# marian42/shapegan

Measured on AMD Instinct MI355X. Metric: GAN train steps/sec @32^3 voxels (train_wgan.py 5 critic + 1 generator updates, batch 64/GPU), higher is better.
Workload: dtype f32; 1 GPU; train_wgan.py 32^3 voxel WGAN, fp32, batch=64 synthetic SDF grids (BASELINE configs[1]); global_batch=64, per_gpu_batch=64, parallelism=dp1

## Files before the change

### shapegan_amd/csrc/conv3d_halo.hip

```cpp
#include "conv_common.h"

#ifndef SG_RING
#define SG_RING 8
#endif
#ifndef SG_ABLATE
#define SG_ABLATE 0
#endif

namespace sg {

constexpr int kHD = 4, kHH = 18, kHWF = 18;
constexpr int kHWH = 10;
constexpr int kROWH = 2 * kHWH;
constexpr int kROWD = kHH * kROWH;
constexpr int kHS = kHD * kROWD;
constexpr int kCC = 4;

struct HaloFwdArgs {
    const float* x;
    const float4* wp;
    const float* bias;
    float* y;
    ConvGeom g;
    int Cin, Cout;
// ... 567 lines not shown

    const int tid = threadIdx.x, lane = tid & 63;
    const int wave = __builtin_amdgcn_readfirstlane(tid >> 6);
    const int wm = R32 ? 0 : wave >> 1, wn = wave & 1, r = lane & 31, kpar = lane >> 5;
    const int tnf = R32 ? wave >> 1 : 0;
    const int lpart = MODE == 0 ? (r >> 3) * BX::BW + (r & 7) : (r >> 4) * BX::PL + ((r >> 2) & 3) * BX::BW + (r & 3);
    const int lanebase = wn * BX::WNOFF + tnf * BX::TNOFF + lpart + 1 - kpar;

    f32x16 acc[NTN];
#pragma unroll
    for (int t = 0; t < NTN; ++t)
#pragma unroll
        for (int q = 0; q < 16; ++q) acc[t][q] = 0.f;

    lds_float* const bl = (lds_float*)box;
    const lds_float* bb[2][kDCC];
#pragma unroll
    for (int b = 0; b < 2; ++b)
#pragma unroll
        for (int c = 0; c < kDCC; ++c) {
            bb[b][c] = bl + b * kDBUF + c * kDB + lanebase;
            pin_vgpr(bb[b][c]);
        }
    lds_float* sdst = bl + tid;
    pin_vgpr(sdst);

    const int G = a.Cout;
    const int par0 = blockIdx.z * a.ppw, par_end = par0 + a.ppw;
    const unsigned par_bytes = (unsigned)(a.mtiles * 2) * (unsigned)G * 1024u;
    const __amdgpu_buffer_rsrc_t wres = make_rsrc(a.wp + ((long)(R32 ? blockIdx.y : blockIdx.y * 2 + wm) * G) * 64);
    const unsigned wvoff = lane * 16;

    const int O3 = a.g.OD * a.g.OH * a.g.OW;
    const int obias = (a.g.OH + 1) * a.g.OW + 1;
    const __amdgpu_buffer_rsrc_t dres = __builtin_amdgcn_make_buffer_rsrc(
        const_cast<float*>(a.dy + (long)n * a.g.Cy * O3 - obias), 0, 1 << 26, 0x00020000);
    const unsigned chan_bytes = (unsigned)O3 * 4u;
    unsigned gword[kDNF], goff[kDNF];
#pragma unroll
    for (int f = 0; f < kDNF; ++f) {
        const int e = tid + 256 * f;
        const int ci = e / kDB;
        int rem = e - ci * kDB, smp = 0;
        if (MODE == 1) {
            smp = rem / 125;
            rem -= smp * 125;
        }
        const int hd = rem / BX::PL, hh = (rem - hd * BX::PL) / BX::BW, hw = rem % BX::BW;
        const int od = qd0 - 1 + hd, oh = qh0 - 1 + hh, ow = qw0 - 1 + hw;
        const bool never = e >= kDCC * kDB || (int)n + smp >= a.batch;
        const unsigned cls = (od < 0 ? 1u << 26 : 0u) | (od + 1 >= a.g.OD ? 1u << 27 : 0u) | (oh < 0 ? 1u << 28 : 0u) |
                             (oh + 1 >= a.g.OH ? 1u << 29 : 0u) | (ow < 0 ? 1u << 30 : 0u) | (ow + 1 >= a.g.OW ? 1u << 31 : 0u);
        const int off0 = (smp * a.g.Cy + ci) * O3 + (od * a.g.OH + oh) * a.g.OW + ow + obias;
        gword[f] = never ? 0xffffffffu : ((unsigned)off0 * 4u) | cls;
        pin_vgpr(gword[f]);
    }
    unsigned pshift = 0;
    auto set_goff = [&](int par) __attribute__((always_inline)) {
        const int pd = (par >> 2) & 1, ph = (par >> 1) & 1, pw = par & 1;
        const unsigned mask = 0x03ffffffu | (pd ? 1u << 27 : 1u << 26) | (ph ? 1u << 29 : 1u << 28) | (pw ? 1u << 31 : 1u << 30);
#pragma unroll
        for (int f = 0; f < kDNF; ++f) goff[f] = gword[f] & mask;
        pshift = (unsigned)((pd * a.g.OH + ph) * a.g.OW + pw) * 4u;
    };
    const long I3 = (long)a.g.ID * a.g.IH * a.g.IW;
    const int nn = MODE == 0 ? (int)n : (int)n + wn;
    const __amdgpu_buffer_rsrc_t ores = make_rsrc(a.dx + (long)(nn < a.batch ? nn : 0) * a.g.Cx * I3);
    const __amdgpu_buffer_rsrc_t bres = make_rsrc(a.bias ? a.bias : a.dx);
    unsigned ovoff[NTN];
#pragma unroll
    for (int tn = 0; tn < NTN; ++tn) {
        int qd, qh, qw;
        if (MODE == 0) {
            qd = qd0 + wn;
            qh = qh0 + (tnf + tn) * 4 + (r >> 3);
            qw = qw0 + (r & 7);
        } else {
            qd = 2 * (tnf + tn) + (r >> 4);
            qh = (r >> 2) & 3;
            qw = r & 3;
        }
        ovoff[tn] = (unsigned)(((2 * qd) * a.g.IH + 2 * qh) * a.g.IW + 2 * qw + 4 * kpar * (int)I3) * 4u;
        pin_vgpr(ovoff[tn]);
    }
    const unsigned bvoff = kpar * 16;
#ifdef SG_DGRAD_NO_PAIR
    const bool paired = false;
#else
    const bool paired = a.ppw >= 2;
#endif
    float keep[NTN][16];
#pragma unroll
    for (int t = 0; t < NTN; ++t)
#pragma unroll
        for (int q = 0; q < 16; ++q) keep[t][q] = 0.f;
    auto write_parity = [&](int par) __attribute__((always_inline)) {
        const int pd = (par >> 2) & 1, ph = (par >> 1) & 1, pw = par & 1;
        const unsigned oshift = (unsigned)((pd * a.g.IH + ph) * a.g.IW) * 4u;
        if (nn < a.batch) {
            if (paired && pw == 0) {
#pragma unroll
                for (int q = 0; q < 16; ++q) {
                    const int cis = ci0 + wm * 32 + (q & 3) + 8 * (q >> 2);
                    const float bv = a.bias && cis < a.Cin ? buf_load(bres, bvoff, (unsigned)cis * 4u) : 0.f;
#pragma unroll
                    for (int tn = 0; tn < NTN; ++tn) keep[tn][q] = sg_apply_act(acc[tn][q] + bv, a.act, a.slope);
                }
            } else if (paired) {
                typedef unsigned u32x2 __attribute__((ext_vector_type(2)));
#pragma unroll
                for (int q = 0; q < 16; ++q) {
                    const int cis = ci0 + wm * 32 + (q & 3) + 8 * (q >> 2);
                    if (cis < a.Cin) {
                        const float bv = a.bias ? buf_load(bres, bvoff, (unsigned)cis * 4u) : 0.f;
#pragma unroll
                        for (int tn = 0; tn < NTN; ++tn) {
                            u32x2 v;
                            v.x = __builtin_bit_cast(unsigned, keep[tn][q]);
                            v.y = __builtin_bit_cast(unsigned, sg_apply_act(acc[tn][q] + bv, a.act, a.slope));
                            __builtin_amdgcn_raw_buffer_store_b64(v, ores, (int)ovoff[tn], (int)((unsigned)cis * (unsigned)I3 * 4u + oshift), 0);
                        }
                    }
                }
            } else {
#pragma unroll
                for (int q = 0; q < 16; ++q) {
                    const int cis = ci0 + wm * 32 + (q & 3) + 8 * (q >> 2);
                    if (cis < a.Cin) {
                        const float bv = a.bias ? buf_load(bres, bvoff, (unsigned)cis * 4u) : 0.f;
#pragma unroll
                        for (int tn = 0; tn < NTN; ++tn) {
                            const float v = sg_apply_act(acc[tn][q] + bv, a.act, a.slope);
                            __builtin_amdgcn_raw_buffer_store_b32(__builtin_bit_cast(unsigned, v), ores, (int)ovoff[tn],
                                                                  (int)((unsigned)cis * (unsigned)I3 * 4u + oshift + 4u * pw), 0);
                        }
                    }
                }
            }
        }
#pragma unroll
        for (int t = 0; t < NTN; ++t)
#pragma unroll
            for (int q = 0; q < 16; ++q) acc[t][q] = 0.f;
    };

    set_goff(par0);
    float fv[kDNF];
    constexpr int kRing = 8;
    float4 aring[kRing];
    unsigned wcur = (unsigned)par0 * par_bytes;
#pragma unroll
    for (int f = 0; f < kDNF; ++f) fv[f] = buf_load(dres, goff[f], pshift);
#pragma unroll
    for (int u = 0; u < kRing; ++u) aring[u] = buf_load4(wres, wvoff, wcur + (unsigned)u * 1024u);
#pragma unroll
    for (int f = 0; f < kDNF; ++f) sdst[256 * f] = fv[f];
    __syncthreads();

    constexpr int O00 = BX::PL + BX::BW, O01 = BX::PL, O10 = BX::BW, O11 = 0;
    const int nstage = a.Cout / kDCC;
    auto stage = [&](auto tag, unsigned dys, unsigned wnext) __attribute__((always_inline)) {
        constexpr int CUR = decltype(tag)::value, NXT = CUR ^ 1;
        float bq[NTN][4];
#pragma unroll
        for (int tn = 0; tn < NTN; ++tn) {
            const lds_float* hb = bb[CUR][0] + tn * BX::TNOFF;
            bq[tn][0] = hb[O00];
            bq[tn][1] = hb[O01];
            bq[tn][2] = hb[O10];
            bq[tn][3] = hb[O11];
        }
        __builtin_amdgcn_sched_barrier(0);
#pragma unroll
        for (int c = 0; c < kDCC; ++c) {
            const float4 a_cur = aring[c % kRing];
            aring[c % kRing] = c + kRing < kDCC ? buf_load4(wres, wvoff, wcur + (unsigned)(c + kRing) * 1024u)
                                                : buf_load4(wres, wvoff, wnext + (unsigned)(c + kRing - kDCC) * 1024u);
            float b[NTN][4];
#pragma unroll
            for (int tn = 0; tn < NTN; ++tn)
#pragma unroll
                for (int j = 0; j < 4; ++j) b[tn][j] = bq[tn][j];
            if (c + 1 < kDCC) {
#pragma unroll
                for (int tn = 0; tn < NTN; ++tn) {
                    const lds_float* hb = bb[CUR][c + 1] + tn * BX::TNOFF;
                    bq[tn][0] = hb[O00];
                    bq[tn][1] = hb[O01];
                    bq[tn][2] = hb[O10];
                    bq[tn][3] = hb[O11];
                }
            }
            if (c < kDCC / 2) {
#pragma unroll
                for (int f = 2 * c; f < 2 * c + 2; ++f) fv[f] = buf_load(dres, goff[f], dys + pshift);
            } else {
#pragma unroll
                for (int f = 2 * (c - kDCC / 2); f < 2 * (c - kDCC / 2) + 2; ++f) sdst[NXT * kDBUF + 256 * f] = fv[f];
            }
            __builtin_amdgcn_sched_barrier(0);
            const float av[4] = {a_cur.x, a_cur.y, a_cur.z, a_cur.w};
#pragma unroll
            for (int j = 0; j < 4; ++j)
#pragma unroll
                for (int tn = 0; tn < NTN; ++tn) acc[tn] = __builtin_amdgcn_mfma_f32_32x32x2f32(av[j], b[tn][j], acc[tn], 0, 0, 0);
            __builtin_amdgcn_sched_barrier(0);
        }
        wcur = wnext;
        __syncthreads();
    };
    for (int par = par0; par < par_end; ++par) {
        const bool more = par + 1 < par_end;
        const unsigned wlast = more ? (unsigned)(par + 1) * par_bytes : (unsigned)par * par_bytes + (unsigned)(nstage - 1) * kDCC * 1024u;
        const unsigned dlast = more ? 0u : (unsigned)(nstage - 1) * kDCC * chan_bytes;
        int s = 0;
        for (; s + 1 < nstage; s += 2) {
            stage(IntTag<0>(), (unsigned)(s + 1) * kDCC * chan_bytes, wcur + kDCC * 1024u);
            const bool last = s + 2 == nstage;
            if (last && more) set_goff(par + 1);
            stage(IntTag<1>(), last ? dlast : (unsigned)(s + 2) * kDCC * chan_bytes, last ? wlast : wcur + kDCC * 1024u);
        }
        if (s < nstage) stage(IntTag<0>(), dlast, wlast);
        write_parity(par);
    }
}

template <int MODE>
__global__ void __launch_bounds__(256) conv_dgrad_halo_kernel(HaloDgradArgs a) {
    conv_dgrad_halo_body<MODE, false>(a);
}
template <int MODE>
__global__ void __launch_bounds__(256) conv_dgrad_halo32_kernel(HaloDgradArgs a) {
    conv_dgrad_halo_body<MODE, true>(a);
}

size_t halo_dgrad_workspace_bytes(int Cin, int Cout) { return (size_t)8 * ((Cin + 63) / 64) * 64 * Cout * 8 * sizeof(float); }

int halo_dgrad_try(const float* dy, const float* w, const float* bias, float* dx, int batch, int Cin, int Cin_total,
                   const ConvGeom& g, int Cout, int act, float slope, void* workspace, size_t workspace_bytes,
                   hipStream_t stream, int force, bool packed_already, PackJobs* collect) {
    const bool mode1 = g.OD == 4 && g.OH == 4 && g.OW == 4;
    if (!mode1 && (g.OW % 8 != 0 || g.OH % 8 != 0 || g.OD % 2 != 0)) return 0;
    if (Cout % 16 != 0 || Cin < 32 || Cin % 8 != 0) return 0;
    if (((long)2 * g.Cy * g.OD * g.OH * g.OW + (long)(g.OH + 1) * g.OW + 1) * 4 >= (1L << 26)) return 0;
    if (!workspace || workspace_bytes < halo_dgrad_workspace_bytes(Cin, Cout)) return 0;
    if ((long)batch * g.Cy * g.OD * g.OH * g.OW >= (1L << 31)) return 0;
    if ((long)2 * g.Cy * g.OD * g.OH * g.OW * 4 >= (long)kBufRange || (long)Cout * 1024 >= (long)kBufRange) return 0;
    const int ntw = mode1 ? 1 : g.OW / 8, nth = mode1 ? 1 : g.OH / 8, ntd = mode1 ? 1 : g.OD / 2;
    const long tiles = mode1 ? (batch + 1) / 2 : (long)batch * ntd * nth * ntw;
    const int mtiles = (Cin + 63) / 64;
    if (!force && tiles * mtiles * 8 < (mode1 ? 16 : 64)) return 0;
    if (tiles >= (1L << 31) || mtiles > 65535) return 0;
    float4* wp = (float4*)workspace;
    if ((long)8 * mtiles * 2 * Cout * 1024 >= (long)kBufRange) return 0;
    if (collect) return collect->add(1, w, wp, Cout, Cin_total, Cin, mtiles * 2);
    if (!packed_already) {
        const long total = 8L * mtiles * 2 * Cout * 64;
        int blocks = (int)((total + 255) / 256);
        if (blocks > 4096) blocks = 4096;
        hipLaunchKernelGGL(pack_dgrad_frag_kernel, dim3(blocks), dim3(256), 0, stream, w, wp, Cout, Cin_total, Cin, mtiles * 2);
    }
    HaloDgradArgs a;
    a.dy = dy;
    a.wp = wp;
    a.bias = bias;
    a.dx = dx;
    a.g = g;
    a.Cin = Cin;
    a.Cout = Cout;
    a.mtiles = mtiles;
    a.batch = batch;
    a.dntw = FastDiv(ntw);
    a.dnth = FastDiv(nth);
    a.dntd = FastDiv(ntd);
    a.act = act;
    a.slope = slope;
    int ppw = 8;
    while (ppw > 1 && (tiles * mtiles * (8 / ppw) < 512 || (force & 2) || (Cout / 16) % 2 != 0)) ppw >>= 1;
    if ((force >> 2) && (Cout / 16) % 2 == 0) ppw = force >> 2;
    if ((long)8 * mtiles * 2 * Cout * 1024 >= (long)kBufRange) return 0;
    a.ppw = ppw;
    size_t lds = (size_t)2 * 16 * 256 * sizeof(float);
    {
        const long wgs = tiles * mtiles * (8 / ppw);
        const long cost2 = ((wgs + 511) / 512) * 2, cost3 = ((wgs + 767) / 768) * 3;
        if (cost2 <= cost3) lds = 56 * 1024;
    }
    const bool r32 = Cin <= 32 || tiles * mtiles * (8 / ppw) < 256;
    const dim3 grid((unsigned)tiles, r32 ? (unsigned)((Cin + 31) / 32) : (unsigned)mtiles, 8 / ppw);
    if (mode1 && r32)
        hipLaunchKernelGGL((conv_dgrad_halo32_kernel<1>), grid, dim3(256), lds, stream, a);
    else if (mode1)
        hipLaunchKernelGGL((conv_dgrad_halo_kernel<1>), grid, dim3(256), lds, stream, a);
    else if (r32)
        hipLaunchKernelGGL((conv_dgrad_halo32_kernel<0>), grid, dim3(256), lds, stream, a);
    else
        hipLaunchKernelGGL((conv_dgrad_halo_kernel<0>), grid, dim3(256), lds, stream, a);
    return 1;
}

constexpr int kWROWD = 368;
constexpr int kWHS = kHD * kWROWD;
constexpr int kWNF = (2 * kHD * kHH + 7) / 8;

struct HaloWgradArgs {
    const float4* ap;
    const float* x;
    float* ws;
    ConvGeom g;
    int Cin, Cout, nslice, per_split, mt_total;
    long ldw;
    FastDiv dntw, dnth, dOD;
};

__global__ void __launch_bounds__(256) pack_wgrad_dy_kernel(const float* __restrict__ dy, float4* __restrict__ ap,
                                                            ConvGeom g, int Cout, int MT, int nslice, FastDiv dntw,
                                                            FastDiv dnth, FastDiv dOD) {
    const long total = (long)MT * nslice * 8 * 64;
    const long O3 = (long)g.OD * g.OH * g.OW;
    for (long e = (long)blockIdx.x * 256 + threadIdx.x; e < total; e += (long)gridDim.x * 256) {
        const int lane = (int)(e & 63);
        const int gq = (int)((e >> 6) & 7);
        const long q = e >> 9;
        const uint32_t sl = (uint32_t)(q % nslice);
        const int mt = (int)(q / nslice);
        uint32_t twi, thi, od, n, q1, q2;
        dntw.divmod(sl, q1, twi);
        dnth.divmod(q1, q2, thi);
        dOD.divmod(q2, n, od);
        const int co = mt * 32 + (lane & 31);
        float4 v = make_float4(0.f, 0.f, 0.f, 0.f);
        if (co < Cout) {
            const float* src = dy + ((long)n * Cout + co) * O3 + ((long)od * g.OH + (thi * 8 + gq)) * g.OW + twi * 8 + (lane >> 5);
            v = make_float4(src[0], src[2], src[4], src[6]);
        }
        ap[e] = v;
    }
}

template <int NCH>
__global__ void __launch_bounds__(256) conv_wgrad_halo_kernel(HaloWgradArgs a) {
    extern __shared__ __attribute__((aligned(16))) float wbox[];
    const int tid = threadIdx.x, lane = tid & 63;
    const int wave = __builtin_amdgcn_readfirstlane(tid >> 6);
    const int wm = NCH == 2 ? wave >> 1 : 0, wn = NCH == 2 ? wave & 1 : wave, r = lane & 31, kpar = lane >> 5;
    const int ci0 = blockIdx.x * NCH;
    const int mt0 = blockIdx.y * (NCH == 2 ? 4 : 2);
    constexpr int NF = NCH == 2 ? kWNF : 2 * kWNF;
    constexpr int NV = NCH == 2 ? kWNF : kWNF / 2;
    const int split = blockIdx.z;
    const int s_beg = split * a.per_split, s_end = min(a.nslice, s_beg + a.per_split);

    int lanebase[2];
#pragma unroll
    for (int tn = 0; tn < 2; ++tn) {
        const int col = wn * 64 + tn * 32 + r;
        const int tap = col & 63, kd = tap >> 4, kh = (tap >> 2) & 3, kw = tap & 3;
        lanebase[tn] = (col >> 6) * kWHS + kd * kWROWD + kh * kROWH + (kw & 1) * kHWH + (kw >> 1) + kpar;
    }

    f32x16 acc[2][2];
#pragma unroll
    for (int i = 0; i < 2; ++i)
#pragma unroll
        for (int j = 0; j < 2; ++j)
#pragma unroll
            for (int q = 0; q < 16; ++q) acc[i][j][q] = 0.f;

    const int I3 = a.g.ID * a.g.IH * a.g.IW;
    const int fl_w = tid & 31, frow = tid >> 5;
    const int lds_w = (fl_w & 1) * kHWH + (fl_w >> 1);
    const int prow = (tid >> 1) % (kHD * kHH);
    const int pad = (prow / kHH) * kWROWD + (prow % kHH) * kROWH + (tid & 1) * kHWH + (kHWH - 1);
    lds_float* const wl = (lds_float*)wbox;
    lds_float* sdst[kWNF / 2];
    unsigned voff[NV], cls[NV];
#pragma unroll
    for (int f = 0; f < kWNF / 2; ++f) {
        const int row = 8 * f + frow;
        const int hd = row / kHH, hh = row - hd * kHH;
        const bool inbox = fl_w < kHWF && row < kHD * kHH;
        sdst[f] = wl + (inbox ? hd * kWROWD + hh * kROWH + lds_w : pad);
        pin_vgpr(sdst[f]);
#pragma unroll
        for (int c = 0; c < (NCH == 2 ? 2 : 1); ++c) {
            const bool ok = inbox && (ci0 + c) < a.Cin;
            voff[c * (kWNF / 2) + f] = ok ? (unsigned)(c * I3 + (hd * a.g.IH + hh) * a.g.IW + fl_w) * 4u : kBufOutside;
            cls[c * (kWNF / 2) + f] = (hd == 0 ? 1u << 26 : 0u) | (hd == kHD - 1 ? 1u << 27 : 0u) | (hh == 0 ? 1u << 28 : 0u) |
                                      (hh == kHH - 1 ? 1u << 29 : 0u) | (fl_w == 0 ? 1u << 30 : 0u) |
                                      (fl_w == kHWF - 1 ? 1u << 31 : 0u);
            pin_vgpr(voff[c * (kWNF / 2) + f]);
            pin_vgpr(cls[c * (kWNF / 2) + f]);
        }
    }
    float fv[NF];
    unsigned eoff[NV];
    __amdgpu_buffer_rsrc_t xres;
    auto xres_of = [&]() __attribute__((always_inline)) { return xres; };
    const unsigned chan_bytes = (unsigned)I3 * 4u;
    auto copy_load = [&](int f) __attribute__((always_inline)) {
        if constexpr (NCH == 2) {
            return buf_load(xres_of(), eoff[f], 0);
        } else {
            return buf_load(xres_of(), eoff[f % (kWNF / 2)], (unsigned)(f / (kWNF / 2)) * chan_bytes);
        }
    };
    const int ntw_ = (int)a.g.OW / 8, nth_ = (int)a.g.OH / 8;
    auto copy_prepare = [&](int sl) {
        uint32_t twi, thi, od, n, q1, q2;
        a.dntw.divmod((uint32_t)sl, q1, twi);
        a.dnth.divmod(q1, q2, thi);
        a.dOD.divmod(q2, n, od);
        const long origin = ((long)n * a.g.Cx + ci0) * I3 + ((2 * (long)od - 1) * a.g.IH + (16 * (long)thi - 1)) * a.g.IW +
                            (16 * (long)twi - 1);
        xres = __builtin_amdgcn_make_buffer_rsrc(const_cast<float*>(a.x + origin), 0, 1 << 26, 0x00020000);
        const unsigned flags = (od == 0 ? 1u << 26 : 0u) | ((int)od == a.g.OD - 1 ? 1u << 27 : 0u) | (thi == 0 ? 1u << 28 : 0u) |
                               ((int)thi == nth_ - 1 ? 1u << 29 : 0u) | (twi == 0 ? 1u << 30 : 0u) |
                               ((int)twi == ntw_ - 1 ? 1u << 31 : 0u);
#pragma unroll
        for (int f = 0; f < NV; ++f) eoff[f] = (cls[f] & flags) | voff[f];
    };

    const int nst = s_end - s_beg;
    constexpr int kRing = 8;
    const int G = nst * 8;
    if (nst > 0) {
        __amdgpu_buffer_rsrc_t ares[2];
#pragma unroll
        for (int t = 0; t < 2; ++t) ares[t] = make_rsrc(a.ap + ((long)(mt0 + wm * 2 + t) * a.nslice + s_beg) * 8 * 64);
        const unsigned avoff = lane * 16;
        const lds_float* bb[2][2][2];
#pragma unroll
        for (int b = 0; b < 2; ++b)
#pragma unroll
            for (int tn = 0; tn < 2; ++tn)
#pragma unroll
                for (int h = 0; h < 2; ++h) {
                    bb[b][tn][h] = wl + b * (NCH * kWHS) + lanebase[tn] + h * (8 * kROWH);
                    pin_vgpr(bb[b][tn][h]);
                }

        copy_prepare(s_beg);
#pragma unroll
        for (int f = 0; f < NF; ++f) fv[f] = copy_load(f);
        float4 aring[kRing][2];
#pragma unroll
        for (int u = 0; u < kRing; ++u)
#pragma unroll
            for (int t = 0; t < 2; ++t) aring[u][t] = buf_load4(ares[t], avoff, (unsigned)(u < G ? u : G - 1) * 1024u);
#pragma unroll
        for (int f = 0; f < NF; ++f) sdst[f % (kWNF / 2)][(f / (kWNF / 2)) * kWHS] = fv[f];
        __syncthreads();

        auto stage = [&](auto tag, int st) {
            constexpr int CUR = decltype(tag)::value, NXT = CUR ^ 1;
            const int snext = st + 1 < nst ? st + 1 : st;
            float bq[2][4];
#pragma unroll
            for (int tn = 0; tn < 2; ++tn) {
                const lds_float* hb = bb[CUR][tn][0];
                bq[tn][0] = hb[0];
                bq[tn][1] = hb[2];
                bq[tn][2] = hb[4];
                bq[tn][3] = hb[6];
            }
            copy_prepare(s_beg + snext);
            __builtin_amdgcn_sched_barrier(0);
#pragma unroll
            for (int gq = 0; gq < 8; ++gq) {
                float4 a_cur[2];
#pragma unroll
                for (int t = 0; t < 2; ++t) a_cur[t] = aring[gq][t];
                int gi = (st + 1) * 8 + gq;
                gi = gi < G ? gi : G - 1;
#pragma unroll
                for (int t = 0; t < 2; ++t) aring[gq][t] = buf_load4(ares[t], avoff, (unsigned)gi * 1024u);
                float b[2][4];
#pragma unroll
                for (int tn = 0; tn < 2; ++tn)
#pragma unroll
                    for (int j = 0; j < 4; ++j) b[tn][j] = bq[tn][j];
                if (gq + 1 < 8) {
#pragma unroll
                    for (int tn = 0; tn < 2; ++tn) {
                        const lds_float* hb = bb[CUR][tn][(gq + 1) >> 2] + 2 * ((gq + 1) & 3) * kROWH;
                        bq[tn][0] = hb[0];
                        bq[tn][1] = hb[2];
                        bq[tn][2] = hb[4];
                        bq[tn][3] = hb[6];
                    }
                }
#pragma unroll
                for (int f = 0; f < NF; ++f) {
                    if (f * 4 / NF == gq) fv[f] = copy_load(f);
                    if (f * 4 / NF + 4 == gq) sdst[f % (kWNF / 2)][NXT * (NCH * kWHS) + (f / (kWNF / 2)) * kWHS] = fv[f];
                }
                __builtin_amdgcn_sched_barrier(0);
#pragma unroll
                for (int j = 0; j < 4; ++j) {
                    const float a0 = j == 0 ? a_cur[0].x : (j == 1 ? a_cur[0].y : (j == 2 ? a_cur[0].z : a_cur[0].w));
                    const float a1 = j == 0 ? a_cur[1].x : (j == 1 ? a_cur[1].y : (j == 2 ? a_cur[1].z : a_cur[1].w));
                    acc[0][0] = __builtin_amdgcn_mfma_f32_32x32x2f32(a0, b[0][j], acc[0][0], 0, 0, 0);
                    acc[1][0] = __builtin_amdgcn_mfma_f32_32x32x2f32(a1, b[0][j], acc[1][0], 0, 0, 0);
                    acc[0][1] = __builtin_amdgcn_mfma_f32_32x32x2f32(a0, b[1][j], acc[0][1], 0, 0, 0);
                    acc[1][1] = __builtin_amdgcn_mfma_f32_32x32x2f32(a1, b[1][j], acc[1][1], 0, 0, 0);
                }
                __builtin_amdgcn_sched_barrier(0);
            }
            __syncthreads();
        };
        for (int st = 0; st + 1 < nst; st += 2) {
            stage(IntTag<0>(), st);
            stage(IntTag<1>(), st + 1);
        }
        if (nst & 1) stage(IntTag<0>(), nst - 1);
    }

    float* out = a.ws + (long)split * a.Cout * a.ldw;
#pragma unroll
    for (int tn = 0; tn < 2; ++tn) {
        const int col = wn * 64 + tn * 32 + r;
        const int ci = ci0 + (col >> 6);
        if (ci >= a.Cin) continue;
        const long cbase = (long)ci * 64 + (col & 63);
#pragma unroll
        for (int t = 0; t < 2; ++t) {
#pragma unroll
            for (int q = 0; q < 16; ++q) {
                const int co = (mt0 + wm * 2 + t) * 32 + (q & 3) + 8 * (q >> 2) + 4 * kpar;
                if (co < a.Cout) out[(long)co * a.ldw + cbase] = acc[t][tn][q];
            }
        }
    }
}

__global__ void __launch_bounds__(256) pack_wgrad_dy4_kernel(const float* __restrict__ dy, float4* __restrict__ ap, int Cout,
                                                             int MT, int nslice) {
    const long total = (long)MT * nslice * 8 * 64;
    for (long e = (long)blockIdx.x * 256 + threadIdx.x; e < total; e += (long)gridDim.x * 256) {
        const int lane = (int)(e & 63);
        const int gq = (int)((e >> 6) & 7);
        const long q = e >> 9;
        const long sl = q % nslice;
        const int mt = (int)(q / nslice);
        const int co = mt * 32 + (lane & 31);
        float4 v = make_float4(0.f, 0.f, 0.f, 0.f);
        if (co < Cout) {
            const float* src = dy + (sl * Cout + co) * 64 + (gq >> 1) * 16 + (gq & 1) * 8 + (lane >> 5);
            v = make_float4(src[0], src[2], src[4], src[6]);
        }
        ap[e] = v;
    }
}

__global__ void __launch_bounds__(256) conv_wgrad_halo4_kernel(HaloWgradArgs a) {
    constexpr int kBUF = 2 * k4CH;
    extern __shared__ __attribute__((aligned(16))) float wbox[];
    lds_float* const wl = (lds_float*)wbox;
    const int tid = threadIdx.x, lane = tid & 63;
    const int wave = __builtin_amdgcn_readfirstlane(tid >> 6);
    const int wm = wave >> 1, wn = wave & 1, r = lane & 31, kpar = lane >> 5;
    const int ci0 = blockIdx.x * 2, mt0 = blockIdx.y * 4, split = blockIdx.z;
    const int s_beg = split * a.per_split, s_end = min(a.nslice, s_beg + a.per_split);
    const int nst = s_end - s_beg;

    f32x16 acc[2][2];
#pragma unroll
    for (int i = 0; i < 2; ++i)
#pragma unroll
        for (int j = 0; j < 2; ++j)
#pragma unroll
            for (int q = 0; q < 16; ++q) acc[i][j][q] = 0.f;

    for (int e = tid; e < 2 * kBUF; e += 256) wl[e] = 0.f;

    if (nst > 0) {
        const lds_float* bb[2][2][4];
#pragma unroll
        for (int tn = 0; tn < 2; ++tn) {
            const int tap = tn * 32 + r, kd = tap >> 4, kh = (tap >> 2) & 3, kw = tap & 3;
            const int lb = wn * k4CH + kd * k4PLANE + kh * k4ROW + (kw & 1) * k4HALF + (kw >> 1) + kpar;
#pragma unroll
            for (int b = 0; b < 2; ++b)
#pragma unroll
                for (int od = 0; od < 4; ++od) {
                    bb[b][tn][od] = wl + b * kBUF + lb + od * (2 * k4PLANE);
                    pin_vgpr(bb[b][tn][od]);
                }
        }
        unsigned voff[4];
        lds_float* sdst[4];
#pragma unroll
        for (int f = 0; f < 4; ++f) {
            const int e = tid + 256 * f, c = e >> 9, idx = e & 511;
            const int id = idx >> 6, ih = (idx >> 3) & 7, iw = idx & 7;
            voff[f] = (ci0 + c) < a.Cin ? (unsigned)e * 4u : kBufOutside;
            sdst[f] = wl + c * k4CH + (id + 1) * k4PLANE + (ih + 1) * k4ROW + ((iw + 1) & 1) * k4HALF + ((iw + 1) >> 1);
            pin_vgpr(voff[f]);
            pin_vgpr(sdst[f]);
        }
        __amdgpu_buffer_rsrc_t ares[2];
#pragma unroll
        for (int t = 0; t < 2; ++t) ares[t] = make_rsrc(a.ap + ((long)(mt0 + wm * 2 + t) * a.nslice + s_beg) * 8 * 64);
        const unsigned avoff = lane * 16;
        const long slice_floats = (long)a.g.Cx * 512;
        const float* xb = a.x + (long)s_beg * slice_floats + (long)ci0 * 512;
        const int G = nst * 8;
        constexpr int kRing = 8;
        float fv[4];
        __syncthreads();
        {
            const __amdgpu_buffer_rsrc_t xres = make_rsrc(xb);
#pragma unroll
            for (int f = 0; f < 4; ++f) fv[f] = buf_load(xres, voff[f], 0);
        }
        float4 aring[kRing][2];
#pragma unroll
        for (int u = 0; u < kRing; ++u)
#pragma unroll
            for (int t = 0; t < 2; ++t) aring[u][t] = buf_load4(ares[t], avoff, (unsigned)(u < G ? u : G - 1) * 1024u);
#pragma unroll
        for (int f = 0; f < 4; ++f) *sdst[f] = fv[f];
        __syncthreads();

        auto stage = [&](auto tag, int st) {
            constexpr int CUR = decltype(tag)::value, NXT = CUR ^ 1;
            const int snext = st + 1 < nst ? st + 1 : st;
            const __amdgpu_buffer_rsrc_t xres = make_rsrc(xb + (long)snext * slice_floats);
            float bq[2][4];
#pragma unroll
            for (int tn = 0; tn < 2; ++tn) {
                const lds_float* hb = bb[CUR][tn][0];
                bq[tn][0] = hb[0];
                bq[tn][1] = hb[2];
                bq[tn][2] = hb[2 * k4ROW];
                bq[tn][3] = hb[2 * k4ROW + 2];
            }
            __builtin_amdgcn_sched_barrier(0);
#pragma unroll
            for (int gq = 0; gq < 8; ++gq) {
                float4 a_cur[2];
#pragma unroll
                for (int t = 0; t < 2; ++t) a_cur[t] = aring[gq][t];
                int gi = (st + 1) * 8 + gq;
                gi = gi < G ? gi : G - 1;
#pragma unroll
                for (int t = 0; t < 2; ++t) aring[gq][t] = buf_load4(ares[t], avoff, (unsigned)gi * 1024u);
                float b[2][4];
#pragma unroll
                for (int tn = 0; tn < 2; ++tn)
#pragma unroll
                    for (int j = 0; j < 4; ++j) b[tn][j] = bq[tn][j];
                if (gq + 1 < 8) {
#pragma unroll
                    for (int tn = 0; tn < 2; ++tn) {
                        const lds_float* hb = bb[CUR][tn][(gq + 1) >> 1] + ((gq + 1) & 1) * (4 * k4ROW);
                        bq[tn][0] = hb[0];
                        bq[tn][1] = hb[2];
                        bq[tn][2] = hb[2 * k4ROW];
                        bq[tn][3] = hb[2 * k4ROW + 2];
                    }
                }
                if (gq < 4) fv[gq] = buf_load(xres, voff[gq], 0);
                else sdst[gq - 4][NXT * kBUF] = fv[gq - 4];
                __builtin_amdgcn_sched_barrier(0);
#pragma unroll
                for (int j = 0; j < 4; ++j) {
                    const float a0 = j == 0 ? a_cur[0].x : (j == 1 ? a_cur[0].y : (j == 2 ? a_cur[0].z : a_cur[0].w));
                    const float a1 = j == 0 ? a_cur[1].x : (j == 1 ? a_cur[1].y : (j == 2 ? a_cur[1].z : a_cur[1].w));
                    acc[0][0] = __builtin_amdgcn_mfma_f32_32x32x2f32(a0, b[0][j], acc[0][0], 0, 0, 0);
                    acc[1][0] = __builtin_amdgcn_mfma_f32_32x32x2f32(a1, b[0][j], acc[1][0], 0, 0, 0);
                    acc[0][1] = __builtin_amdgcn_mfma_f32_32x32x2f32(a0, b[1][j], acc[0][1], 0, 0, 0);
                    acc[1][1] = __builtin_amdgcn_mfma_f32_32x32x2f32(a1, b[1][j], acc[1][1], 0, 0, 0);
                }
                __builtin_amdgcn_sched_barrier(0);
            }
            __syncthreads();
        };
        for (int st = 0; st + 1 < nst; st += 2) {
            stage(IntTag<0>(), st);
            stage(IntTag<1>(), st + 1);
        }
        if (nst & 1) stage(IntTag<0>(), nst - 1);
    }

    float* out = a.ws + (long)split * a.Cout * a.ldw;
#pragma unroll
    for (int tn = 0; tn < 2; ++tn) {
        const int col = wn * 64 + tn * 32 + r;
        const int ci = ci0 + (col >> 6);
        if (ci >= a.Cin) continue;
        const long cbase = (long)ci * 64 + (col & 63);
#pragma unroll
        for (int t = 0; t < 2; ++t) {
#pragma unroll
            for (int q = 0; q < 16; ++q) {
                const int co = (mt0 + wm * 2 + t) * 32 + (q & 3) + 8 * (q >> 2) + 4 * kpar;
                if (co < a.Cout) out[(long)co * a.ldw + cbase] = acc[t][tn][q];
            }
        }
    }
}

__global__ void __launch_bounds__(256) wgrad_halo_finalize_kernel(const float* __restrict__ ws, float* __restrict__ dw,
                                                                  int Cout, int ncol, long ldw, int nsplit) {
    const long total = (long)Cout * ncol, total4 = total >> 2;
    for (long e4 = (long)blockIdx.x * 256 + threadIdx.x; e4 < total4; e4 += (long)gridDim.x * 256) {
        const f32x4* p = reinterpret_cast<const f32x4*>(ws) + e4;
        f32x4 v = {0.f, 0.f, 0.f, 0.f};
        int s = 0;
        for (; s + 3 < nsplit; s += 4) {
            const f32x4 a0 = p[(long)s * total4], a1 = p[(long)(s + 1) * total4], a2 = p[(long)(s + 2) * total4],
                        a3 = p[(long)(s + 3) * total4];
            v += a0;
            v += a1;
            v += a2;
            v += a3;
        }
        for (; s < nsplit; ++s) v += p[(long)s * total4];
        const long e = e4 << 2;
        const long co = e / ncol, c = e - co * ncol;
        *reinterpret_cast<f32x4*>(dw + co * ldw + c) = v;
    }
}

static bool wgrad_mode4(const ConvGeom& g) { return g.OD == 4 && g.OH == 4 && g.OW == 4; }

static bool wgrad_rows64(const ConvGeom& g, int Cin, int Cout) {
    return !wgrad_mode4(g) && Cout <= 64 && Cin >= 4 && Cin % 4 == 0;
}
static void wgrad_halo_plan(int batch, const ConvGeom& g, int Cin, int Cout, int& nslice, int& nsplit, int& mtiles) {
    nslice = wgrad_mode4(g) ? batch : batch * g.OD * (g.OH / 8) * (g.OW / 8);
    const bool rows64 = wgrad_rows64(g, Cin, Cout);
    mtiles = rows64 ? (Cout + 63) / 64 : (Cout + 127) / 128;
    const int ntiles = (rows64 ? Cin / 4 : (Cin + 1) / 2) * mtiles;
    nsplit = (512 + ntiles - 1) / ntiles;
    if (nsplit > nslice / 4) nsplit = nslice / 4 > 0 ? nslice / 4 : 1;
    if (nsplit < 1) nsplit = 1;
}

size_t halo_wgrad_workspace_bytes(int batch, int Cin, int Cout, int OD, int OH, int OW) {
    if ((OH % 8 != 0 || OW % 8 != 0) && !(OD == 4 && OH == 4 && OW == 4)) return 0;
    ConvGeom g;
    g.OD = OD;
    g.OH = OH;
    g.OW = OW;
    int nslice, nsplit, mtiles;
    g.ID = 2 * OD;
    g.IH = 2 * OH;
    g.IW = 2 * OW;
    wgrad_halo_plan(batch, g, Cin, Cout, nslice, nsplit, mtiles);
    const size_t pack = (size_t)mtiles * 4 * nslice * 8 * 64 * sizeof(float4);
    const size_t part = (size_t)nsplit * Cout * Cin * 64 * sizeof(float);
    return pack + part + 256;
}

int halo_wgrad_dy_image_plan(int batch, int Cin, int Cout, const ConvGeom& g, size_t workspace_bytes, int* mt_total, long* nslice_out) {
    const bool mode4 = wgrad_mode4(g);
    if (!(mode4 || (g.OD == 8 && g.OH == 8 && g.OW == 8)) || Cout % 128 != 0 || Cin < 2) return 0;
    if ((long)batch * g.Cx * g.ID * g.IH * g.IW >= (1L << 31) || (long)2 * g.ID * g.IH * g.IW * 4 >= (1L << 26)) return 0;
    int nslice, nsplit, mtiles;
    wgrad_halo_plan(batch, g, Cin, Cout, nslice, nsplit, mtiles);
    const int ntiles = ((Cin + 1) / 2) * mtiles;
    if (Cout <= 64 || (long)ntiles * nsplit < 384) return 0;
    if (workspace_bytes < halo_wgrad_workspace_bytes(batch, Cin, Cout, g.OD, g.OH, g.OW)) return 0;
    *mt_total = mtiles * 4;
    *nslice_out = nslice;
    return 1;
}

__global__ void __launch_bounds__(256) act_bwd_pack8_kernel(const float* __restrict__ y, const float* __restrict__ dy,
                                                            float* __restrict__ dz, float* __restrict__ rowsum,
                                                            float4* __restrict__ ap, long rows, int C, long nslice, int act, float slope) {
    const long row = (long)blockIdx.x * 4 + (threadIdx.x >> 6);
    if (row >= rows) return;
    const int lane = threadIdx.x & 63;
    const long base = row * 512 + lane * 8;
    const f32x4 y0 = *reinterpret_cast<const f32x4*>(y + base), y1 = *reinterpret_cast<const f32x4*>(y + base + 4);
    const f32x4 g0 = *reinterpret_cast<const f32x4*>(dy + base), g1 = *reinterpret_cast<const f32x4*>(dy + base + 4);
    f32x4 z0, z1;
#pragma unroll
    for (int j = 0; j < 4; ++j) {
        z0[j] = act == SG_ACT_LEAKY ? (y0[j] > 0.f ? g0[j] : g0[j] * slope) : (y0[j] > 0.f ? g0[j] : 0.f);
        z1[j] = act == SG_ACT_LEAKY ? (y1[j] > 0.f ? g1[j] : g1[j] * slope) : (y1[j] > 0.f ? g1[j] : 0.f);
    }
    *reinterpret_cast<f32x4*>(dz + base) = z0;
    *reinterpret_cast<f32x4*>(dz + base + 4) = z1;
    const float s = sg_wave_sum(((z0[0] + z0[1]) + (z0[2] + z0[3])) + ((z1[0] + z1[1]) + (z1[2] + z1[3])));
    if (lane == 0) rowsum[row] = s;
    const long n = row / C;
    const int co = (int)(row - n * C), mt = co >> 5, r = co & 31, od = lane >> 3, oh = lane & 7;
    const long e = (((long)mt * nslice + n * 8 + od) * 8 + oh) * 64 + r;
    ap[e] = make_float4(z0[0], z0[2], z1[0], z1[2]);
    ap[e + 32] = make_float4(z0[1], z0[3], z1[1], z1[3]);
}
int halo_act_bwd_pack8_launch(const float* y, const float* dy, float* dz, float* rowsum, void* ap, long rows, int C, long nslice,
                              int act, float slope, hipStream_t stream) {
    hipLaunchKernelGGL(act_bwd_pack8_kernel, dim3((unsigned)((rows + 3) / 4)), dim3(256), 0, stream, y, dy, dz, rowsum, (float4*)ap,
                       rows, C, nslice, act, slope);
    return 1;
}

int halo_wgrad_try(const float* dy, const float* x, float* dw, int batch, int Cin, int Cin_total, const ConvGeom& g, int Cout,
                   void* workspace, size_t workspace_bytes, hipStream_t stream, int force, bool dy_packed) {
    const bool mode4 = wgrad_mode4(g);
    if ((!mode4 && (g.OW % 8 != 0 || g.OH % 8 != 0)) || Cin < 2 || Cout < 32) return 0;
    if ((long)batch * g.Cx * g.ID * g.IH * g.IW >= (1L << 31)) return 0;
    if ((long)2 * g.ID * g.IH * g.IW * 4 >= (1L << 26)) return 0;
    int nslice, nsplit, mtiles;
    wgrad_halo_plan(batch, g, Cin, Cout, nslice, nsplit, mtiles);
    const bool rows64 = wgrad_rows64(g, Cin, Cout) && (long)4 * g.ID * g.IH * g.IW * 4 < (1L << 26);
    if (wgrad_rows64(g, Cin, Cout) && !rows64) return 0;
    const int ntiles = (rows64 ? Cin / 4 : (Cin + 1) / 2) * mtiles;
    if (!force && ((Cout <= 64 && !rows64) || (long)ntiles * nsplit < 384)) return 0;
    const size_t need = halo_wgrad_workspace_bytes(batch, Cin, Cout, g.OD, g.OH, g.OW);
    if (!workspace || workspace_bytes < need) return 0;
    const int per_split = (nslice + nsplit - 1) / nsplit;
    nsplit = (nslice + per_split - 1) / per_split;

    const FastDiv dntw(mode4 ? 1 : g.OW / 8), dnth(mode4 ? 1 : g.OH / 8), dOD(g.OD);
    float4* ap = (float4*)workspace;
    const size_t pack_floats4 = (size_t)mtiles * 4 * nslice * 8 * 64;
    float* part = (float*)(ap + pack_floats4);
    if (!dy_packed) {
        int blocks = (int)((pack_floats4 + 255) / 256);
        if (blocks > 8192) blocks = 8192;
        if (mode4)
            hipLaunchKernelGGL(pack_wgrad_dy4_kernel, dim3(blocks), dim3(256), 0, stream, dy, ap, Cout, mtiles * 4, nslice);
        else
            hipLaunchKernelGGL(pack_wgrad_dy_kernel, dim3(blocks), dim3(256), 0, stream, dy, ap, g, Cout, rows64 ? mtiles * 2 : mtiles * 4,
                               nslice, dntw, dnth, dOD);
    }
    HaloWgradArgs a;
    a.ap = ap;
    a.x = x;
    a.g = g;
    a.Cin = Cin;
    a.Cout = Cout;
    a.nslice = nslice;
    a.per_split = per_split;
    a.mt_total = rows64 ? mtiles * 2 : mtiles * 4;
    a.dntw = dntw;
    a.dnth = dnth;
    a.dOD = dOD;
    const bool direct = nsplit == 1;
    a.ws = direct ? dw : part;
    a.ldw = direct ? (long)Cin_total * 64 : (long)Cin * 64;
    if (mode4) {
        hipLaunchKernelGGL(conv_wgrad_halo4_kernel, dim3((Cin + 1) / 2, mtiles, nsplit), dim3(256),
                           (size_t)2 * 2 * k4CH * sizeof(float), stream, a);
    } else {
        if (rows64) {
            const size_t lds = (size_t)2 * 4 * kWHS * sizeof(float);
            hipLaunchKernelGGL(conv_wgrad_halo_kernel<4>, dim3(Cin / 4, mtiles, nsplit), dim3(256), lds, stream, a);
        } else {
            const size_t lds = (size_t)2 * 2 * kWHS * sizeof(float);
            hipLaunchKernelGGL(conv_wgrad_halo_kernel<2>, dim3((Cin + 1) / 2, mtiles, nsplit), dim3(256), lds, stream, a);
        }
    }
    if (!direct) {
        const long total = (long)Cout * Cin * 64;
        int fb = (int)((total / 4 + 255) / 256);
        if (fb > 2048) fb = 2048;
        hipLaunchKernelGGL(wgrad_halo_finalize_kernel, dim3(fb), dim3(256), 0, stream, (const float*)part, dw, Cout, Cin * 64,
                           (long)Cin_total * 64, nsplit);
    }
    return 1;
}

}
```

Before: 60.34 steps/s.

## Remap wgrad columns so waves skip padding-only MFMA steps statically

Reorders the weight-gradient GEMM column-to-tap mapping in the halo wgrad kernels so that each wave-pair owns a fixed group of kernel-depth taps. This lets the boundary steps that touch only zero padding be skipped at compile time: both their LDS B loads and their MFMAs are dropped. The 2-channel path gets a specialised variant for OH==8, with a smaller LDS row stride and boundary flags folded into the buffer offsets. The mode-4 kernel is always specialised this way. The cost is two instantiated bodies per kernel with a wave-level branch, plus remapped output indexing that must stay correct.

```diff
diff --git a/shapegan_amd/csrc/conv3d_halo.hip b/shapegan_amd/csrc/conv3d_halo.hip
--- a/shapegan_amd/csrc/conv3d_halo.hip
+++ b/shapegan_amd/csrc/conv3d_halo.hip
@@ -893,6 +893,7 @@
 constexpr int kWROWD = 368;
 constexpr int kWHS = kHD * kWROWD;
 constexpr int kWNF = (2 * kHD * kHH + 7) / 8;
+constexpr int kWROWD_SKIP = 364;
 
 struct HaloWgradArgs {
     const float4* ap;
@@ -929,12 +930,16 @@
     }
 }
 
-template <int NCH>
-__global__ void __launch_bounds__(256) conv_wgrad_halo_kernel(HaloWgradArgs a) {
+template <int NCH, int V>
+__device__ __forceinline__ void conv_wgrad_halo_body(const HaloWgradArgs& a) {
+    constexpr bool SKIP = V >= 0;
+    static_assert(!SKIP || NCH == 2, "the static-skip column map is the 2-channel form's");
+    constexpr int WROWD = SKIP ? kWROWD_SKIP : kWROWD;
+    constexpr int WHS = kHD * WROWD;
     extern __shared__ __attribute__((aligned(16))) float wbox[];
     const int tid = threadIdx.x, lane = tid & 63;
     const int wave = __builtin_amdgcn_readfirstlane(tid >> 6);
-    const int wm = NCH == 2 ? wave >> 1 : 0, wn = NCH == 2 ? wave & 1 : wave, r = lane & 31, kpar = lane >> 5;
+    const int wm = NCH == 2 ? wave >> 1 : 0, wn = SKIP ? V : (NCH == 2 ? wave & 1 : wave), r = lane & 31, kpar = lane >> 5;
     const int ci0 = blockIdx.x * NCH;
     const int mt0 = blockIdx.y * (NCH == 2 ? 4 : 2);
     constexpr int NF = NCH == 2 ? kWNF : 2 * kWNF;
@@ -942,12 +947,13 @@
     const int split = blockIdx.z;
     const int s_beg = split * a.per_split, s_end = min(a.nslice, s_beg + a.per_split);
 
+    auto col_ci = [&](int tn) { return SKIP ? r >> 4 : (wn * 64 + tn * 32 + r) >> 6; };
+    auto col_tap = [&](int tn) { return SKIP ? ((r >> 2) & 3) * 16 + (2 * wn + tn) * 4 + (r & 3) : (tn * 32 + r) & 63; };
     int lanebase[2];
 #pragma unroll
     for (int tn = 0; tn < 2; ++tn) {
-        const int col = wn * 64 + tn * 32 + r;
-        const int tap = col & 63, kd = tap >> 4, kh = (tap >> 2) & 3, kw = tap & 3;
-        lanebase[tn] = (col >> 6) * kWHS + kd * kWROWD + kh * kROWH + (kw & 1) * kHWH + (kw >> 1) + kpar;
+        const int tap = col_tap(tn), kd = tap >> 4, kh = (tap >> 2) & 3, kw = tap & 3;
+        lanebase[tn] = col_ci(tn) * WHS + kd * WROWD + kh * kROWH + (kw & 1) * kHWH + (kw >> 1) + kpar;
     }
 
     f32x16 acc[2][2];
@@ -962,7 +968,7 @@
     const int fl_w = tid & 31, frow = tid >> 5;
     const int lds_w = (fl_w & 1) * kHWH + (fl_w >> 1);
     const int prow = (tid >> 1) % (kHD * kHH);
-    const int pad = (prow / kHH) * kWROWD + (prow % kHH) * kROWH + (tid & 1) * kHWH + (kHWH - 1);
+    const int pad = (prow / kHH) * WROWD + (prow % kHH) * kROWH + (tid & 1) * kHWH + (kHWH - 1);
     lds_float* const wl = (lds_float*)wbox;
     lds_float* sdst[kWNF / 2];
     unsigned voff[NV], cls[NV];
@@ -971,7 +977,7 @@
         const int row = 8 * f + frow;
         const int hd = row / kHH, hh = row - hd * kHH;
         const bool inbox = fl_w < kHWF && row < kHD * kHH;
-        sdst[f] = wl + (inbox ? hd * kWROWD + hh * kROWH + lds_w : pad);
+        sdst[f] = wl + (inbox ? hd * WROWD + hh * kROWH + lds_w : pad);
         pin_vgpr(sdst[f]);
 #pragma unroll
         for (int c = 0; c < (NCH == 2 ? 2 : 1); ++c) {
@@ -980,8 +986,12 @@
             cls[c * (kWNF / 2) + f] = (hd == 0 ? 1u << 26 : 0u) | (hd == kHD - 1 ? 1u << 27 : 0u) | (hh == 0 ? 1u << 28 : 0u) |
                                       (hh == kHH - 1 ? 1u << 29 : 0u) | (fl_w == 0 ? 1u << 30 : 0u) |
                                       (fl_w == kHWF - 1 ? 1u << 31 : 0u);
+            if constexpr (SKIP) {
+                voff[c * (kWNF / 2) + f] = ok ? voff[c * (kWNF / 2) + f] | cls[c * (kWNF / 2) + f] : 1u << 28;
+            } else {
+                pin_vgpr(cls[c * (kWNF / 2) + f]);
+            }
             pin_vgpr(voff[c * (kWNF / 2) + f]);
-            pin_vgpr(cls[c * (kWNF / 2) + f]);
         }
     }
     float fv[NF];
@@ -1009,7 +1019,7 @@
                                ((int)thi == nth_ - 1 ? 1u << 29 : 0u) | (twi == 0 ? 1u << 30 : 0u) |
                                ((int)twi == ntw_ - 1 ? 1u << 31 : 0u);
 #pragma unroll
-        for (int f = 0; f < NV; ++f) eoff[f] = (cls[f] & flags) | voff[f];
+        for (int f = 0; f < NV; ++f) eoff[f] = SKIP ? voff[f] & (flags | 0x03ffffffu) : (cls[f] & flags) | voff[f];
     };
 
     const int nst = s_end - s_beg;
@@ -1021,15 +1031,26 @@
         for (int t = 0; t < 2; ++t) ares[t] = make_rsrc(a.ap + ((long)(mt0 + wm * 2 + t) * a.nslice + s_beg) * 8 * 64);
         const unsigned avoff = lane * 16;
         const lds_float* bb[2][2][2];
-#pragma unroll
-        for (int b = 0; b < 2; ++b)
-#pragma unroll
-            for (int tn = 0; tn < 2; ++tn)
-#pragma unroll
-                for (int h = 0; h < 2; ++h) {
-                    bb[b][tn][h] = wl + b * (NCH * kWHS) + lanebase[tn] + h * (8 * kROWH);
-                    pin_vgpr(bb[b][tn][h]);
-                }
+        if constexpr (SKIP) {
+            const lds_float* b0 = wl + lanebase[0];
+            pin_vgpr(b0);
+#pragma unroll
+            for (int b = 0; b < 2; ++b)
+#pragma unroll
+                for (int tn = 0; tn < 2; ++tn)
+#pragma unroll
+                    for (int h = 0; h < 2; ++h) bb[b][tn][h] = b0 + b * (NCH * WHS) + tn * kROWH + h * (8 * kROWH);
+        } else {
+#pragma unroll
+            for (int b = 0; b < 2; ++b)
+#pragma unroll
+                for (int tn = 0; tn < 2; ++tn)
+#pragma unroll
+                    for (int h = 0; h < 2; ++h) {
+                        bb[b][tn][h] = wl + b * (NCH * WHS) + lanebase[tn] + h * (8 * kROWH);
+                        pin_vgpr(bb[b][tn][h]);
+                    }
+        }
 
         copy_prepare(s_beg);
 #pragma unroll
@@ -1040,15 +1061,17 @@
 #pragma unroll
             for (int t = 0; t < 2; ++t) aring[u][t] = buf_load4(ares[t], avoff, (unsigned)(u < G ? u : G - 1) * 1024u);
 #pragma unroll
-        for (int f = 0; f < NF; ++f) sdst[f % (kWNF / 2)][(f / (kWNF / 2)) * kWHS] = fv[f];
+        for (int f = 0; f < NF; ++f) sdst[f % (kWNF / 2)][(f / (kWNF / 2)) * WHS] = fv[f];
         __syncthreads();
 
         auto stage = [&](auto tag, int st) {
             constexpr int CUR = decltype(tag)::value, NXT = CUR ^ 1;
+            auto dead = [](int tn, int gq) { return (V == 0 && tn == 0 && gq == 0) || (V == 1 && tn == 1 && gq == 7); };
             const int snext = st + 1 < nst ? st + 1 : st;
-            float bq[2][4];
+            float bq[2][4] = {};
 #pragma unroll
             for (int tn = 0; tn < 2; ++tn) {
+                if (dead(tn, 0)) continue;
                 const lds_float* hb = bb[CUR][tn][0];
                 bq[tn][0] = hb[0];
                 bq[tn][1] = hb[2];
@@ -1074,6 +1097,7 @@
                 if (gq + 1 < 8) {
 #pragma unroll
                     for (int tn = 0; tn < 2; ++tn) {
+                        if (dead(tn, gq + 1)) continue;
                         const lds_float* hb = bb[CUR][tn][(gq + 1) >> 2] + 2 * ((gq + 1) & 3) * kROWH;
                         bq[tn][0] = hb[0];
                         bq[tn][1] = hb[2];
@@ -1084,17 +1108,21 @@
 #pragma unroll
                 for (int f = 0; f < NF; ++f) {
                     if (f * 4 / NF == gq) fv[f] = copy_load(f);
-                    if (f * 4 / NF + 4 == gq) sdst[f % (kWNF / 2)][NXT * (NCH * kWHS) + (f / (kWNF / 2)) * kWHS] = fv[f];
+                    if (f * 4 / NF + 4 == gq) sdst[f % (kWNF / 2)][NXT * (NCH * WHS) + (f / (kWNF / 2)) * WHS] = fv[f];
                 }
                 __builtin_amdgcn_sched_barrier(0);
 #pragma unroll
                 for (int j = 0; j < 4; ++j) {
                     const float a0 = j == 0 ? a_cur[0].x : (j == 1 ? a_cur[0].y : (j == 2 ? a_cur[0].z : a_cur[0].w));
                     const float a1 = j == 0 ? a_cur[1].x : (j == 1 ? a_cur[1].y : (j == 2 ? a_cur[1].z : a_cur[1].w));
-                    acc[0][0] = __builtin_amdgcn_mfma_f32_32x32x2f32(a0, b[0][j], acc[0][0], 0, 0, 0);
-                    acc[1][0] = __builtin_amdgcn_mfma_f32_32x32x2f32(a1, b[0][j], acc[1][0], 0, 0, 0);
-                    acc[0][1] = __builtin_amdgcn_mfma_f32_32x32x2f32(a0, b[1][j], acc[0][1], 0, 0, 0);
-                    acc[1][1] = __builtin_amdgcn_mfma_f32_32x32x2f32(a1, b[1][j], acc[1][1], 0, 0, 0);
+                    if (!dead(0, gq)) {
+                        acc[0][0] = __builtin_amdgcn_mfma_f32_32x32x2f32(a0, b[0][j], acc[0][0], 0, 0, 0);
+                        acc[1][0] = __builtin_amdgcn_mfma_f32_32x32x2f32(a1, b[0][j], acc[1][0], 0, 0, 0);
+                    }
+                    if (!dead(1, gq)) {
+                        acc[0][1] = __builtin_amdgcn_mfma_f32_32x32x2f32(a0, b[1][j], acc[0][1], 0, 0, 0);
+                        acc[1][1] = __builtin_amdgcn_mfma_f32_32x32x2f32(a1, b[1][j], acc[1][1], 0, 0, 0);
+                    }
                 }
                 __builtin_amdgcn_sched_barrier(0);
             }
@@ -1110,10 +1138,9 @@
     float* out = a.ws + (long)split * a.Cout * a.ldw;
 #pragma unroll
     for (int tn = 0; tn < 2; ++tn) {
-        const int col = wn * 64 + tn * 32 + r;
-        const int ci = ci0 + (col >> 6);
+        const int ci = ci0 + col_ci(tn);
         if (ci >= a.Cin) continue;
-        const long cbase = (long)ci * 64 + (col & 63);
+        const long cbase = (long)ci * 64 + col_tap(tn);
 #pragma unroll
         for (int t = 0; t < 2; ++t) {
 #pragma unroll
@@ -1125,6 +1152,17 @@
     }
 }
 
+template <int NCH, bool SKIP = false>
+__global__ void __launch_bounds__(256) conv_wgrad_halo_kernel(HaloWgradArgs a) {
+    if constexpr (!SKIP) {
+        conv_wgrad_halo_body<NCH, -1>(a);
+    } else {
+        if ((__builtin_amdgcn_readfirstlane(threadIdx.x >> 6) & 1) == 0) conv_wgrad_halo_body<NCH, 0>(a);
+        else conv_wgrad_halo_body<NCH, 1>(a);
+    }
+}
+
+constexpr int kW4HALF = 6, kW4ROW = 12, kW4PLANE = 120, kW4CH = 10 * kW4PLANE;
 __global__ void __launch_bounds__(256) pack_wgrad_dy4_kernel(const float* __restrict__ dy, float4* __restrict__ ap, int Cout,
                                                              int MT, int nslice) {
     const long total = (long)MT * nslice * 8 * 64;
@@ -1144,13 +1182,14 @@
     }
 }
 
-__global__ void __launch_bounds__(256) conv_wgrad_halo4_kernel(HaloWgradArgs a) {
-    constexpr int kBUF = 2 * k4CH;
+template <int V>
+__device__ __forceinline__ void conv_wgrad_halo4_body(const HaloWgradArgs& a) {
+    constexpr int kBUF = 2 * kW4CH;
     extern __shared__ __attribute__((aligned(16))) float wbox[];
     lds_float* const wl = (lds_float*)wbox;
     const int tid = threadIdx.x, lane = tid & 63;
     const int wave = __builtin_amdgcn_readfirstlane(tid >> 6);
-    const int wm = wave >> 1, wn = wave & 1, r = lane & 31, kpar = lane >> 5;
+    const int wm = wave >> 1, wn = V, r = lane & 31, kpar = lane >> 5;
     const int ci0 = blockIdx.x * 2, mt0 = blockIdx.y * 4, split = blockIdx.z;
     const int s_beg = split * a.per_split, s_end = min(a.nslice, s_beg + a.per_split);
     const int nst = s_end - s_beg;
@@ -1169,13 +1208,13 @@
         const lds_float* bb[2][2][4];
 #pragma unroll
         for (int tn = 0; tn < 2; ++tn) {
-            const int tap = tn * 32 + r, kd = tap >> 4, kh = (tap >> 2) & 3, kw = tap & 3;
-            const int lb = wn * k4CH + kd * k4PLANE + kh * k4ROW + (kw & 1) * k4HALF + (kw >> 1) + kpar;
+            const int kd = 2 * wn + tn, kh = (r >> 2) & 3, kw = r & 3;
+            const int lb = (r >> 4) * kW4CH + kd * kW4PLANE + kh * kW4ROW + (kw & 1) * kW4HALF + (kw >> 1) + kpar;
 #pragma unroll
             for (int b = 0; b < 2; ++b)
 #pragma unroll
                 for (int od = 0; od < 4; ++od) {
-                    bb[b][tn][od] = wl + b * kBUF + lb + od * (2 * k4PLANE);
+                    bb[b][tn][od] = wl + b * kBUF + lb + od * (2 * kW4PLANE);
                     pin_vgpr(bb[b][tn][od]);
                 }
         }
@@ -1186,7 +1225,7 @@
             const int e = tid + 256 * f, c = e >> 9, idx = e & 511;
             const int id = idx >> 6, ih = (idx >> 3) & 7, iw = idx & 7;
             voff[f] = (ci0 + c) < a.Cin ? (unsigned)e * 4u : kBufOutside;
-            sdst[f] = wl + c * k4CH + (id + 1) * k4PLANE + (ih + 1) * k4ROW + ((iw + 1) & 1) * k4HALF + ((iw + 1) >> 1);
+            sdst[f] = wl + c * kW4CH + (id + 1) * kW4PLANE + (ih + 1) * kW4ROW + ((iw + 1) & 1) * kW4HALF + ((iw + 1) >> 1);
             pin_vgpr(voff[f]);
             pin_vgpr(sdst[f]);
         }
@@ -1216,16 +1255,18 @@
 
         auto stage = [&](auto tag, int st) {
             constexpr int CUR = decltype(tag)::value, NXT = CUR ^ 1;
+            auto dead = [](int tn, int gq) { return (V == 0 && tn == 0 && gq < 2) || (V == 1 && tn == 1 && gq >= 6); };
             const int snext = st + 1 < nst ? st + 1 : st;
             const __amdgpu_buffer_rsrc_t xres = make_rsrc(xb + (long)snext * slice_floats);
-            float bq[2][4];
+            float bq[2][4] = {};
 #pragma unroll
             for (int tn = 0; tn < 2; ++tn) {
+                if (dead(tn, 0)) continue;
                 const lds_float* hb = bb[CUR][tn][0];
                 bq[tn][0] = hb[0];
                 bq[tn][1] = hb[2];
-                bq[tn][2] = hb[2 * k4ROW];
-                bq[tn][3] = hb[2 * k4ROW + 2];
+                bq[tn][2] = hb[2 * kW4ROW];
+                bq[tn][3] = hb[2 * kW4ROW + 2];
             }
             __builtin_amdgcn_sched_barrier(0);
 #pragma unroll
@@ -1245,11 +1286,12 @@
                 if (gq + 1 < 8) {
 #pragma unroll
                     for (int tn = 0; tn < 2; ++tn) {
-                        const lds_float* hb = bb[CUR][tn][(gq + 1) >> 1] + ((gq + 1) & 1) * (4 * k4ROW);
+                        if (dead(tn, gq + 1)) continue;
+                        const lds_float* hb = bb[CUR][tn][(gq + 1) >> 1] + ((gq + 1) & 1) * (4 * kW4ROW);
                         bq[tn][0] = hb[0];
                         bq[tn][1] = hb[2];
-                        bq[tn][2] = hb[2 * k4ROW];
-                        bq[tn][3] = hb[2 * k4ROW + 2];
+                        bq[tn][2] = hb[2 * kW4ROW];
+                        bq[tn][3] = hb[2 * kW4ROW + 2];
                     }
                 }
                 if (gq < 4) fv[gq] = buf_load(xres, voff[gq], 0);
@@ -1259,10 +1301,14 @@
                 for (int j = 0; j < 4; ++j) {
                     const float a0 = j == 0 ? a_cur[0].x : (j == 1 ? a_cur[0].y : (j == 2 ? a_cur[0].z : a_cur[0].w));
                     const float a1 = j == 0 ? a_cur[1].x : (j == 1 ? a_cur[1].y : (j == 2 ? a_cur[1].z : a_cur[1].w));
-                    acc[0][0] = __builtin_amdgcn_mfma_f32_32x32x2f32(a0, b[0][j], acc[0][0], 0, 0, 0);
-                    acc[1][0] = __builtin_amdgcn_mfma_f32_32x32x2f32(a1, b[0][j], acc[1][0], 0, 0, 0);
-                    acc[0][1] = __builtin_amdgcn_mfma_f32_32x32x2f32(a0, b[1][j], acc[0][1], 0, 0, 0);
-                    acc[1][1] = __builtin_amdgcn_mfma_f32_32x32x2f32(a1, b[1][j], acc[1][1], 0, 0, 0);
+                    if (!dead(0, gq)) {
+                        acc[0][0] = __builtin_amdgcn_mfma_f32_32x32x2f32(a0, b[0][j], acc[0][0], 0, 0, 0);
+                        acc[1][0] = __builtin_amdgcn_mfma_f32_32x32x2f32(a1, b[0][j], acc[1][0], 0, 0, 0);
+                    }
+                    if (!dead(1, gq)) {
+                        acc[0][1] = __builtin_amdgcn_mfma_f32_32x32x2f32(a0, b[1][j], acc[0][1], 0, 0, 0);
+                        acc[1][1] = __builtin_amdgcn_mfma_f32_32x32x2f32(a1, b[1][j], acc[1][1], 0, 0, 0);
+                    }
                 }
                 __builtin_amdgcn_sched_barrier(0);
             }
@@ -1278,10 +1324,9 @@
     float* out = a.ws + (long)split * a.Cout * a.ldw;
 #pragma unroll
     for (int tn = 0; tn < 2; ++tn) {
-        const int col = wn * 64 + tn * 32 + r;
-        const int ci = ci0 + (col >> 6);
+        const int ci = ci0 + (r >> 4);
         if (ci >= a.Cin) continue;
-        const long cbase = (long)ci * 64 + (col & 63);
+        const long cbase = (long)ci * 64 + (2 * wn + tn) * 16 + (r & 15);
 #pragma unroll
         for (int t = 0; t < 2; ++t) {
 #pragma unroll
@@ -1291,6 +1336,11 @@
             }
         }
     }
+}
+
+__global__ void __launch_bounds__(256) conv_wgrad_halo4_kernel(HaloWgradArgs a) {
+    if ((__builtin_amdgcn_readfirstlane(threadIdx.x >> 6) & 1) == 0) conv_wgrad_halo4_body<0>(a);
+    else conv_wgrad_halo4_body<1>(a);
 }
 
 __global__ void __launch_bounds__(256) wgrad_halo_finalize_kernel(const float* __restrict__ ws, float* __restrict__ dw,
@@ -1439,14 +1489,19 @@
     a.ldw = direct ? (long)Cin_total * 64 : (long)Cin * 64;
     if (mode4) {
         hipLaunchKernelGGL(conv_wgrad_halo4_kernel, dim3((Cin + 1) / 2, mtiles, nsplit), dim3(256),
-                           (size_t)2 * 2 * k4CH * sizeof(float), stream, a);
+                           (size_t)2 * 2 * kW4CH * sizeof(float), stream, a);
     } else {
         if (rows64) {
             const size_t lds = (size_t)2 * 4 * kWHS * sizeof(float);
-            hipLaunchKernelGGL(conv_wgrad_halo_kernel<4>, dim3(Cin / 4, mtiles, nsplit), dim3(256), lds, stream, a);
+            hipLaunchKernelGGL((conv_wgrad_halo_kernel<4, false>), dim3(Cin / 4, mtiles, nsplit), dim3(256), lds, stream, a);
         } else {
-            const size_t lds = (size_t)2 * 2 * kWHS * sizeof(float);
-            hipLaunchKernelGGL(conv_wgrad_halo_kernel<2>, dim3((Cin + 1) / 2, mtiles, nsplit), dim3(256), lds, stream, a);
+            if (g.OH == 8) {
+                const size_t lds = (size_t)2 * 2 * kHD * kWROWD_SKIP * sizeof(float);
+                hipLaunchKernelGGL((conv_wgrad_halo_kernel<2, true>), dim3((Cin + 1) / 2, mtiles, nsplit), dim3(256), lds, stream, a);
+            } else {
+                const size_t lds = (size_t)2 * 2 * kWHS * sizeof(float);
+                hipLaunchKernelGGL((conv_wgrad_halo_kernel<2, false>), dim3((Cin + 1) / 2, mtiles, nsplit), dim3(256), lds, stream, a);
+            }
         }
     }
     if (!direct) {
```

Result: faster. 61.41 steps/s (median of 6 runs) (+1.8%).
